# afermg/aliby

Measured on AMD Instinct MI355X. Metric: FOV tiles/sec (whole node), higher is better.
Workload: dtype u16 pixels, f64 feature accumulators, f32 dynamics, bfloat16 U-Net

## Files before the change

### aliby_amd/csrc/nn_conv.hip

```cpp
#include "common.h"
#include <utility>

typedef __bf16 bf16x8_t __attribute__((ext_vector_type(8)));
typedef float f32x16_t __attribute__((ext_vector_type(16)));
typedef float f32x2_t __attribute__((ext_vector_type(2)));

namespace {

template <class F, int... I>
__device__ __forceinline__ void static_for_impl(F&& f, std::integer_sequence<int, I...>) {
  (f(std::integral_constant<int, I>{}), ...);
}
template <int N, class F>
__device__ __forceinline__ void static_for(F&& f) {
  static_for_impl(static_cast<F&&>(f), std::make_integer_sequence<int, N>{});
}

__device__ __forceinline__ float cv_bf2f(unsigned h) { return __uint_as_float(h << 16); }
typedef __bf16 bf16x2_t __attribute__((ext_vector_type(2)));
__device__ __forceinline__ unsigned cv_pack2(float lo, float hi) {
  const f32x2_t f = {lo, hi};
  const bf16x2_t b = __builtin_convertvector(f, bf16x2_t);
  return __builtin_bit_cast(unsigned, b);
}
// ... 298 lines not shown
          const int gapi = kb < 32 ? kb + 1 : TW + 2;
          const int bp = lx - 1 - (lx > gapi ? 1 : 0);
          const int snd = bp >= kb ? 1 : 0;
          const int c = snd ? bp - kb : cst + bp;
          const bool ok = lx != gapi && c >= 0 && c < a.W && !(bp == TW && kb == TW) && (unsigned)gy < (unsigned)a.H;
          const int img = (snd && ok) ? g0 + 1 : g0;
          inside |= (unsigned)ok << u;
          later |= (unsigned)snd << u;
          v[u] = inN[(unsigned)(((img * a.H + cy) * IW + min(max(c, 0), a.W - 1)) * a.cs + pl)];
        } else {
          const int gxi = x0 - 1 + lx;
          inside |= (unsigned)((unsigned)gy < (unsigned)a.H && (unsigned)gxi < (unsigned)a.W) << u;
          const int cx = min(max(gxi, 0), a.W - 1);
          v[u] = inN[(unsigned)(((UP ? cy >> 1 : cy) * IW + (UP ? cx >> 1 : cx)) * a.cs + pl)];
        }
      }
#pragma unroll
      for (int u = 0; u < BATCH; ++u) {
        if (it0 + u >= ITERS) break;
        uint4 o;
        if constexpr (PACK) {
          f32x2_t shs[4];
#pragma unroll
          for (int k = 0; k < 4; ++k) shs[k] = ((later >> u) & 1u) ? sh1[k] : sh[k];
          o = conv_act8(v[u], sc, shs, 0u - ((inside >> u) & 1u));
        } else {
          o = conv_act8(v[u], sc, sh, 0u - ((inside >> u) & 1u));
        }
        if (it0 + u == ITERS - 1 && p0 + (it0 + u) * PIX_PER_IT >= RAW) continue;
        lds[pl * PLANE + p0 + (it0 + u) * PIX_PER_IT] = o;
      }
    }
    if constexpr (PK > 0) {
      constexpr int POCT = 2 * PK, PUNITS = TH * TW * POCT;
      const uint4* pN = a.pin + (size_t)n * a.H * a.W * a.pcs;
#pragma unroll
      for (int it = 0; it < (PUNITS + 255) / 256; ++it) {
        const int u = tid + it * 256;
        if (u >= PUNITS) break;
        const int oct = u % POCT, pix = u / POCT;
        const int cy = min(y0 + pix / TW, a.H - 1), cx = min(x0 + pix % TW, a.W - 1);
        uint4 v = make_uint4(0, 0, 0, 0);
        if (oct < a.pcs) v = pN[(unsigned)((cy * a.W + cx) * a.pcs + oct)];
        ldsP[oct * PPLANE + pix] = v;
      }
    }
    CONV_STAMP(3);
    __syncthreads();
    CONV_STAMP(4);

#pragma unroll
    for (int pass = 0; pass < PASSES; ++pass) {
      const int rbase = (rg * PASSES + pass) * R;
      f32x16_t acc[R];
      {
        float4 b4[4];
#pragma unroll
        for (int q = 0; q < 4; ++q) b4[q] = float4(sbias[(c0 >> 2) + q]);
        conv_seed<R>(acc, b4, rr, a.res != nullptr);
      }
      __builtin_amdgcn_sched_barrier(0);
      if (pass + 1 < PASSES && a.res) load_res(pass + 1);
      __builtin_amdgcn_sched_barrier(0);
      conv_mfma<R, KC, (POOL ? cfg::DEPTH_POOL : cfg::DEPTH), PLANE, LW>(
          reinterpret_cast<const bf16x8_t*>(lds) + hh * PLANE + rbase * LW + px + second, wfrag, acc);
      if constexpr (PK > 0) {
        const bf16x8_t* LP = reinterpret_cast<const bf16x8_t*>(ldsP) + hh * PPLANE + rbase * TW + px;
#pragma unroll
        for (int r = 0; r < R; ++r)
#pragma unroll
          for (int k = 0; k < PK; ++k)
            acc[r] = __builtin_amdgcn_mfma_f32_32x32x16_bf16(pfrag[k], LP[2 * k * PPLANE + r * TW], acc[r], 0, 0, 0);
      }
      if (pass == PASSES - 1) CONV_STAMP(5);
      if constexpr (HEAD) {
        __builtin_amdgcn_sched_barrier(0);
#pragma unroll
        for (int r = 0; r < R; ++r) {
          const f32x16_t y = head_from_acc(acc[r], hconst, hconst + 32, hwf, hh);
          const int gy = y0 + rbase + r;
          if (hh == 0 && gx < a.W && gy < a.H) {
            float* hp = a.hout + (size_t)n * a.hO * a.H * a.W + (size_t)gy * a.W + gx;
            const float yo[4] = {y[0], y[1], y[2], y[3]};
            for (int o = 0; o < a.hO; ++o) hp[(size_t)o * a.H * a.W] = yo[o] + hconst[64 + o];
          }
        }
      }
      if (!HEAD || a.out) conv_store<R>(a, nimg, irow, y0 + rbase, gx, c0, acc);
      if constexpr (POOL) {
        const int PH = a.H >> 1, PW = a.W >> 1;
#pragma unroll
        for (int r = 0; r < R; r += 2) {
          const int gy = y0 + rbase + r;
          const bool writer = (px & 1) == 0 && gx + 1 < a.W && gy + 1 < a.H;
          uint4* pp = a.pool + (size_t)nimg * PH * PW * a.ocs + a.ocoff + (unsigned)((((irow + gy) >> 1) * PW + (gx >> 1)) * a.ocs + (c0 >> 3));
#pragma unroll
          for (int half = 0; half < 2; ++half) {
            unsigned pk[4];
#pragma unroll
            for (int q = 0; q < 4; ++q) {
              const float v0 = fmaxf(acc[r][half * 8 + 2 * q], acc[r + 1][half * 8 + 2 * q]);
              const float v1 = fmaxf(acc[r][half * 8 + 2 * q + 1], acc[r + 1][half * 8 + 2 * q + 1]);
              pk[q] = cv_pack2(fmaxf(v0, __shfl_xor(v0, 1)), fmaxf(v1, __shfl_xor(v1, 1)));
            }
            if (writer) pp[half] = make_uint4(pk[0], pk[1], pk[2], pk[3]);
          }
        }
      }
    }
    CONV_STAMP(6);
  }
}

template <int CIN, int COUT, bool UP, bool PACK = false>
struct DmaCfg {
  static constexpr int KC = CIN / 16, NPL = CIN / 8, NCB = COUT / 32;
  static constexpr int WAVES_PER_SIMD = CIN >= 128 ? 1 : 2;
  static constexpr int R = CIN >= 64 ? 2 : 4;
  static constexpr int PASSES = (CIN >= 128 || COUT >= 128) ? 2 : 1;
  static constexpr int RG = 4 / NCB;
  static constexpr int TH = RG * R * PASSES, TW = 32, LH = TH + 2, LW = TW + 2 + (PACK ? 1 : 0);
  static constexpr int RAW = LH * LW;
  static constexpr int PLANE = NPL == 4 ? RAW + (10 - RAW % 8) % 8 : (RAW | 1);
  static constexpr int A_SLOTS = NPL * PLANE;
  static constexpr int PIX_PER_IT = 256 / NPL;
  static constexpr int ITERS = (RAW + PIX_PER_IT - 1) / PIX_PER_IT;
  static constexpr int RLH = UP ? TH / 2 + 2 : LH, RLW = UP ? TW / 2 + 2 : LW;
  static constexpr int RUNITS = RLH * RLW * NPL;
  static constexpr int GIT = (RUNITS + 255) / 256;
  static constexpr int R_SLOTS = GIT * 256;
  static constexpr int LDS_BYTES = (A_SLOTS + R_SLOTS) * 16;
  static constexpr int DEPTH = (CIN >= 64 && COUT >= 64) ? 4 : 6;
};

template <int CIN, int COUT, bool UP, bool PACK = false>
__global__ __launch_bounds__(256, (DmaCfg<CIN, COUT, UP, PACK>::WAVES_PER_SIMD)) void k_conv3x3_dma(ConvArgs a) {
  static_assert(!PACK || UP, "the packed LDS-DMA variant is written for upsampled input");
  using cfg = DmaCfg<CIN, COUT, UP, PACK>;
  constexpr int KC = cfg::KC, NPL = cfg::NPL, NCB = cfg::NCB, R = cfg::R, TH = cfg::TH, TW = cfg::TW;
  constexpr int LW = cfg::LW, RAW = cfg::RAW, PLANE = cfg::PLANE, RLW = cfg::RLW, PASSES = cfg::PASSES;
  constexpr int PIX_PER_IT = cfg::PIX_PER_IT, ITERS = cfg::ITERS, GIT = cfg::GIT;
  extern __shared__ uint4 lds[];
  uint4* const ldsA = lds;
  uint4* const ldsR = lds + cfg::A_SLOTS;

  const int tid = threadIdx.x, lane = tid & 63, wave = tid >> 6;
  const int cb = wave % NCB, rg = wave / NCB;
  const int px = lane & 31, hh = lane >> 5;
  const int c0 = cb * 32 + hh * 16;

  bf16x8_t wfrag[9 * KC];
  {
    const bf16x8_t* wp = reinterpret_cast<const bf16x8_t*>(a.wpk) + (size_t)cb * 9 * KC * 64 + lane;
#pragma unroll
    for (int i = 0; i < 9 * KC; ++i) wfrag[i] = wp[i * 64];
  }
  const int pl = tid % NPL, pix0 = tid / NPL;
  const int ly0 = pix0 / LW, lx0 = pix0 - ly0 * LW;
  f32x2_t sc[4];
#pragma unroll
  for (int k = 0; k < 4; ++k) sc[k] = f32x2_t{a.scale[pl * 8 + 2 * k], a.scale[pl * 8 + 2 * k + 1]};

  const int IH = UP ? a.H >> 1 : a.H, IW = UP ? a.W >> 1 : a.W;
  const int xcd = blockIdx.x & 7, slot = blockIdx.x >> 3, nslots = gridDim.x >> 3;
  const int per_xcd = (a.ntiles + 7) >> 3;
  const int t_end = min(a.ntiles, (xcd + 1) * per_xcd);
  const int wave_u = __builtin_amdgcn_readfirstlane(wave);

  auto issue_dma = [&](int tile) {
    const int tx = tile % a.tiles_x, tyn = tile / a.tiles_x;
    const int ty = tyn % a.tiles_y, n = tyn / a.tiles_y;
    const int ry0 = UP ? (ty * TH >> 1) - 1 : ty * TH - 1, rx0 = UP ? (tx * TW >> 1) - 1 : tx * TW - 1;
    int g0 = 0, cst = 0, half = 1 << 20;
    if constexpr (PACK) {
      g0 = (tx * TW) / a.W;
      cst = tx * TW - g0 * a.W;
      half = (a.W - cst) >> 1;
    }
    const uint4* inN = a.in + (size_t)(PACK ? n * a.G : n) * IH * IW * a.cs + a.coff;
    int t0 = tid;
    asm volatile("" : "+v"(t0));
#pragma unroll
    for (int k = 0; k < GIT; ++k) {
      const int unit = t0 + k * 256;
      const int rpix = unit / NPL, oct = unit % NPL;
      const int rly = rpix / RLW, rlx = rpix - rly * RLW;
      const int iy = min(max(ry0 + rly, 0), IH - 1);
      int ix, img = 0;
      if constexpr (PACK) {
        const bool first = rlx <= half;
        ix = min(max(first ? (cst >> 1) - 1 + rlx : rlx - half - 1, 0), IW - 1);
        img = first ? g0 : min(g0 + 1, a.G - 1);
      } else {
        ix = min(max(rx0 + rlx, 0), IW - 1);
      }
      const uint4* g = inN + (unsigned)(((img * IH + iy) * IW + ix) * a.cs + oct);
      __builtin_amdgcn_global_load_lds((const __attribute__((address_space(1))) void*)g,
                                       (__attribute__((address_space(3))) void*)(ldsR + k * 256 + wave_u * 64), 16, 0, 0);
    }
  };

  int tile = xcd * per_xcd + slot, stamp_tile = 0;
  if (tile < t_end) issue_dma(tile);
  for (; tile < t_end; tile += nslots, ++stamp_tile) {
    CONV_STAMP(0);
    const int tx = tile % a.tiles_x, tyn = tile / a.tiles_x;
    const int ty = tyn % a.tiles_y, n = tyn / a.tiles_y;
    const int y0 = ty * TH, x0 = tx * TW;
    int g0 = 0, cst = x0, kb = 1 << 20, nimg = n;
    if constexpr (PACK) {
      g0 = x0 / a.W;
      cst = x0 - g0 * a.W;
      kb = a.W - cst;
      nimg = n * a.G;
    }
    const int second = (PACK && px >= kb) ? 1 : 0;
    const int gx = PACK ? (second ? px - kb : cst + px) : x0 + px;
    const int irow = PACK ? (g0 + second) * a.H : 0;

    f32x2_t sh[4], sh1[PACK ? 4 : 1];
    {
      const float* sp = a.shift + (size_t)(nimg + g0) * a.shift_stride + pl * 8;
#pragma unroll
      for (int k = 0; k < 4; ++k) sh[k] = f32x2_t{sp[2 * k], sp[2 * k + 1]};
      if constexpr (PACK) {
        const float* sq = a.shift + (size_t)(nimg + min(g0 + 1, a.G - 1)) * a.shift_stride + pl * 8;
#pragma unroll
        for (int k = 0; k < 4; ++k) sh1[k] = f32x2_t{sq[2 * k], sq[2 * k + 1]};
      }
    }
    float4 b4[4] = {};
    if (a.bias) {
      const float4* bp = reinterpret_cast<const float4*>(a.bias + c0);
#pragma unroll
      for (int q = 0; q < 4; ++q) b4[q] = bp[q];
    }
    uint4 rr[R][2];
    auto load_res = [&](int pass) { conv_load_res<R>(a, nimg, irow, y0 + (rg * PASSES + pass) * R, gx, c0, rr); };
    if (a.res) load_res(0);
    CONV_STAMP(1);
    asm volatile("s_waitcnt vmcnt(0)" ::: "memory");
    __syncthreads();
    CONV_STAMP(2);
    {
      const int ry0 = UP ? (y0 >> 1) - 1 : y0 - 1, rx0 = UP ? (x0 >> 1) - 1 : x0 - 1;
      int p0 = pix0, qy = ly0, qx = lx0;
      asm volatile("" : "+v"(p0), "+v"(qy), "+v"(qx));
#pragma unroll
      for (int it = 0; it < ITERS; ++it) {
        int lx = qx + (it * PIX_PER_IT) % LW, ly = qy + (it * PIX_PER_IT) / LW;
        if (lx >= LW) { lx -= LW; ly += 1; }
        const int gy = y0 - 1 + ly, gxi = x0 - 1 + lx;
        const int pix = p0 + it * PIX_PER_IT;
        unsigned keep;
        int rpix;
        uint4 o;
        if constexpr (PACK) {
          const int gapi = kb < 32 ? kb + 1 : TW + 2;
          const int bp = lx - 1 - (lx > gapi ? 1 : 0);
          const int snd = bp >= kb ? 1 : 0;
          const int c = snd ? bp - kb : cst + bp;
          keep = 0u - (unsigned)(lx != gapi && c >= 0 && c < a.W && !(bp == TW && kb == TW) && (unsigned)gy < (unsigned)a.H);
          const int rcol = snd ? (kb >> 1) + 1 + (c >> 1) : ((cst + bp) >> 1) - ((cst >> 1) - 1);
          rpix = min(max(((gy >> 1) - ry0) * RLW + rcol, 0), cfg::RLH * RLW - 1);
          f32x2_t shs[4];
#pragma unroll
          for (int k = 0; k < 4; ++k) shs[k] = snd ? sh1[k] : sh[k];
          o = conv_act8(ldsR[rpix * NPL + pl], sc, shs, keep);
        } else {
          keep = 0u - (unsigned)((unsigned)gy < (unsigned)a.H && (unsigned)gxi < (unsigned)a.W);
          rpix = UP ? min(((gy >> 1) - ry0) * RLW + ((gxi >> 1) - rx0), cfg::RLH * RLW - 1) : min(pix, RAW - 1);
          o = conv_act8(ldsR[rpix * NPL + pl], sc, sh, keep);
        }
        if (it == ITERS - 1 && pix >= RAW) continue;
        ldsA[pl * PLANE + pix] = o;
      }
    }
    CONV_STAMP(3);
    __syncthreads();
#pragma unroll
    for (int pass = 0; pass < PASSES; ++pass) {
      const int rbase = (rg * PASSES + pass) * R;
      f32x16_t acc[R];
      conv_seed<R>(acc, b4, rr, a.res != nullptr);
      __builtin_amdgcn_sched_barrier(0);
      if (pass == 0 && tile + nslots < t_end) issue_dma(tile + nslots);
      if (pass + 1 < PASSES && a.res) load_res(pass + 1);
      __builtin_amdgcn_sched_barrier(0);
      if (pass == 0) CONV_STAMP(4);
      conv_mfma<R, KC, cfg::DEPTH, PLANE, LW>(reinterpret_cast<const bf16x8_t*>(ldsA) + hh * PLANE + rbase * LW + px + second, wfrag, acc);
      if (pass == PASSES - 1) CONV_STAMP(5);
      conv_store<R>(a, nimg, irow, y0 + rbase, gx, c0, acc);
    }
    CONV_STAMP(6);
  }
}

struct PairCfg {
  static constexpr int KC = 2, NPL = 4, R = 2, PASSES = 2;
  static constexpr int TH = 14, TWO = 30, MH = 16, MW = 32, IH = 18, IW = 34;
  static constexpr int RAW_IN = IH * IW, PLANE_IN = RAW_IN + (10 - RAW_IN % 8) % 8;
  static constexpr int RAW_MID = MH * MW, PLANE_MID = RAW_MID + (10 - RAW_MID % 8) % 8;
  static constexpr int PIX_PER_IT = 256 / NPL, ITERS = (RAW_IN + PIX_PER_IT - 1) / PIX_PER_IT;
  static constexpr int MID_SLOTS = NPL * PLANE_MID + 8;
  static constexpr int SLOTS = NPL * PLANE_IN + 2 * MID_SLOTS;
  static constexpr int LDS_BYTES = SLOTS * 16;
  static constexpr int DEPTH = 6;
};

template <bool POOL, bool HEAD>
__global__ __launch_bounds__(512, 1) void k_conv_pair32(ConvArgs a) {
  static_assert(!(POOL && HEAD), "either the pooled output (down block) or the output head (last unit)");
  using cfg = PairCfg;
  constexpr int KC = cfg::KC, NPL = cfg::NPL, R = cfg::R, PASSES = cfg::PASSES, TH = cfg::TH, TWO = cfg::TWO;
  constexpr int IW_ = cfg::IW, MW = cfg::MW, PLANE_IN = cfg::PLANE_IN, PLANE_MID = cfg::PLANE_MID, RAW_IN = cfg::RAW_IN;
  constexpr int PIX_PER_IT = cfg::PIX_PER_IT, ITERS = cfg::ITERS;
  extern __shared__ uint4 lds[];
  uint4* const ldsIn = lds;
  uint4* const ldsMid0 = lds + NPL * PLANE_IN;
  __shared__ __align__(16) float tabB[64];
  __shared__ float hconst[HEAD ? 2 * 32 + 4 : 1];

  const int consumer = threadIdx.x >> 8;
  const int tid = threadIdx.x & 255, lane = tid & 63, wave = tid >> 6;
  const int px = lane & 31, hh = lane >> 5;
  const int c0 = hh * 16;

  const int xcd = blockIdx.x & 7, slot = blockIdx.x >> 3, nslots = gridDim.x >> 3;
  const int per_xcd = (a.ntiles + 7) >> 3;
  const int t_begin = xcd * per_xcd + slot, t_end = min(a.ntiles, (xcd + 1) * per_xcd);
  const int my_tiles = t_begin < t_end ? (t_end - t_begin + nslots - 1) / nslots : 0;

  if (!consumer) {
    bf16x8_t wA[9 * KC];
    {
      const bf16x8_t* pa = reinterpret_cast<const bf16x8_t*>(a.wpk) + lane;
#pragma unroll
      for (int i = 0; i < 9 * KC; ++i) wA[i] = pa[i * 64];
    }
    const int pl = tid % NPL, pix0 = tid / NPL;
    const int ly0 = pix0 / IW_, lx0 = pix0 - ly0 * IW_;
    f32x2_t sc[4];
#pragma unroll
    for (int k = 0; k < 4; ++k) sc[k] = f32x2_t{a.scale[pl * 8 + 2 * k], a.scale[pl * 8 + 2 * k + 1]};
    uint4 v[ITERS];
    unsigned inside = 0;
    auto request = [&](int tile) {
      const int tx = tile % a.tiles_x, tyn = tile / a.tiles_x;
      const int ty = tyn % a.tiles_y, n = tyn / a.tiles_y;
      const int y0 = ty * TH, x0 = tx * TWO;
      const uint4* inN = a.in + (size_t)n * a.H * a.W * a.cs + a.coff;
      inside = 0;
#pragma unroll
      for (int u = 0; u < ITERS; ++u) {
        int lx = lx0 + (u * PIX_PER_IT) % IW_, ly = ly0 + (u * PIX_PER_IT) / IW_;
        if (lx >= IW_) { lx -= IW_; ly += 1; }
        const int gy = y0 - 2 + ly, gxi = x0 - 2 + lx;
        inside |= (unsigned)((unsigned)gy < (unsigned)a.H && (unsigned)gxi < (unsigned)a.W) << u;
        const int cy = min(max(gy, 0), a.H - 1), cx = min(max(gxi, 0), a.W - 1);
        v[u] = inN[(unsigned)((cy * a.W + cx) * a.cs + pl)];
      }
    };
    if (my_tiles > 0) request(t_begin);
    for (int it = 0; it < my_tiles; ++it) {
      const int tile = t_begin + it * nslots;
      const int tx = tile % a.tiles_x, tyn = tile / a.tiles_x;
      const int ty = tyn % a.tiles_y, n = tyn / a.tiles_y;
      const int y0 = ty * TH, x0 = tx * TWO;
      uint4* const ldsMid = ldsMid0 + (it & 1) * cfg::MID_SLOTS;
      f32x2_t sh[4];
      {
        const float* sp = a.shift + (size_t)n * a.shift_stride + pl * 8;
#pragma unroll
        for (int k = 0; k < 4; ++k) sh[k] = f32x2_t{sp[2 * k], sp[2 * k + 1]};
      }
      if (tid < 32) {
        tabB[tid] = a.scale2[tid];
        tabB[32 + tid] = a.shift2[(size_t)n * a.shift2_stride + tid];
      }
#pragma unroll
      for (int u = 0; u < ITERS; ++u) {
        const uint4 o = conv_act8(v[u], sc, sh, 0u - ((inside >> u) & 1u));
        if (u == ITERS - 1 && pix0 + u * PIX_PER_IT >= RAW_IN) continue;
        ldsIn[pl * PLANE_IN + pix0 + u * PIX_PER_IT] = o;
      }
      __syncthreads();
      if (it + 1 < my_tiles) request(tile + nslots);
      __builtin_amdgcn_sched_barrier(0);
#pragma unroll
      for (int pass = 0; pass < PASSES; ++pass) {
        const int mbase = (wave * PASSES + pass) * R;
        f32x16_t acc[R];
        {
          float4 b4[4] = {};
          if (a.bias) {
            const float4* bp = reinterpret_cast<const float4*>(a.bias + c0);
#pragma unroll
            for (int q = 0; q < 4; ++q) b4[q] = bp[q];
          }
#pragma unroll
          for (int r = 0; r < R; ++r)
#pragma unroll
            for (int q = 0; q < 4; ++q) { acc[r][4 * q] = b4[q].x; acc[r][4 * q + 1] = b4[q].y; acc[r][4 * q + 2] = b4[q].z; acc[r][4 * q + 3] = b4[q].w; }
        }
        __builtin_amdgcn_sched_barrier(0);
        conv_mfma<R, KC, cfg::DEPTH, PLANE_IN, IW_>(reinterpret_cast<const bf16x8_t*>(ldsIn) + hh * PLANE_IN + mbase * IW_ + px, wA, acc);
        __builtin_amdgcn_sched_barrier(0);
        const int mgx = x0 - 1 + px;
#pragma unroll
        for (int r = 0; r < R; ++r) {
          const int mgy = y0 - 1 + mbase + r;
          const unsigned keep = 0u - (unsigned)((unsigned)mgy < (unsigned)a.H && (unsigned)mgx < (unsigned)a.W);
#pragma unroll
          for (int half = 0; half < 2; ++half) {
            f32x2_t s2[4], h2[4];
            const float4* tp = reinterpret_cast<const float4*>(tabB + c0 + 8 * half);
            const float4 sa = tp[0], sb = tp[1], ha = tp[8], hb = tp[9];
            s2[0] = f32x2_t{sa.x, sa.y}; s2[1] = f32x2_t{sa.z, sa.w}; s2[2] = f32x2_t{sb.x, sb.y}; s2[3] = f32x2_t{sb.z, sb.w};
            h2[0] = f32x2_t{ha.x, ha.y}; h2[1] = f32x2_t{ha.z, ha.w}; h2[2] = f32x2_t{hb.x, hb.y}; h2[3] = f32x2_t{hb.z, hb.w};
            const uint4 raw = make_uint4(cv_pack2(acc[r][8 * half + 0], acc[r][8 * half + 1]), cv_pack2(acc[r][8 * half + 2], acc[r][8 * half + 3]),
                                         cv_pack2(acc[r][8 * half + 4], acc[r][8 * half + 5]), cv_pack2(acc[r][8 * half + 6], acc[r][8 * half + 7]));
            ldsMid[(2 * hh + half) * PLANE_MID + (mbase + r) * MW + px] = conv_act8(raw, s2, h2, keep);
          }
        }
      }
      __syncthreads();
    }
    __syncthreads();
    __syncthreads();
  } else {
    bf16x8_t wB[9 * KC];
    {
      const bf16x8_t* pb = reinterpret_cast<const bf16x8_t*>(a.wpk2) + lane;
#pragma unroll
      for (int i = 0; i < 9 * KC; ++i) wB[i] = pb[i * 64];
    }
    HeadW hwf;
    if constexpr (HEAD) {
      hwf = head_weights(a.hw, a.hO, lane);
      if (tid < 32) {
        hconst[tid] = a.hscale[tid];
        hconst[32 + tid] = a.hshift[tid];
        if (tid < 4) hconst[64 + tid] = tid < a.hO ? a.hbias[tid] : 0.f;
      }
    }
    float4 b4[4] = {};
    if (a.bias2) {
      const float4* bp = reinterpret_cast<const float4*>(a.bias2 + c0);
#pragma unroll
      for (int q = 0; q < 4; ++q) b4[q] = bp[q];
    }
    __syncthreads();
    __syncthreads();
    for (int it = 0; it < my_tiles; ++it) {
      const int tile = t_begin + it * nslots;
      const int tx = tile % a.tiles_x, tyn = tile / a.tiles_x;
      const int ty = tyn % a.tiles_y, n = tyn / a.tiles_y;
      const int y0 = ty * TH, x0 = tx * TWO;
      const uint4* const ldsMid = ldsMid0 + (it & 1) * cfg::MID_SLOTS;
      const int gx = (px < TWO && x0 + px < a.W) ? x0 + px : a.W;
#pragma unroll
      for (int pass = 0; pass < PASSES; ++pass) {
        const int rbase = (wave * PASSES + pass) * R;
        if (rbase < TH) {
          uint4 rr[R][2];
          if (a.res) conv_load_res<R>(a, n, 0, y0 + rbase, min(gx, a.W - 1), c0, rr);
          f32x16_t acc[R];
          conv_seed<R>(acc, b4, rr, a.res != nullptr);
          __builtin_amdgcn_sched_barrier(0);
          conv_mfma<R, KC, cfg::DEPTH, PLANE_MID, MW>(reinterpret_cast<const bf16x8_t*>(ldsMid) + hh * PLANE_MID + rbase * MW + px, wB, acc);
          if constexpr (HEAD) {
#pragma unroll
            for (int r = 0; r < R; ++r) {
              const f32x16_t y = head_from_acc(acc[r], hconst, hconst + 32, hwf, hh);
              const int gy = y0 + rbase + r;
              if (hh == 0 && gx < a.W && gy < a.H) {
                float* hp = a.hout + (size_t)n * a.hO * a.H * a.W + (size_t)gy * a.W + gx;
                const float yo[4] = {y[0], y[1], y[2], y[3]};
                for (int o = 0; o < a.hO; ++o) hp[(size_t)o * a.H * a.W] = yo[o] + hconst[64 + o];
              }
            }
          }
          if (!HEAD || a.out) conv_store<R>(a, n, 0, y0 + rbase, gx, c0, acc);
          if constexpr (POOL) {
            const int PH = a.H >> 1, PW = a.W >> 1;
            const int gy = y0 + rbase;
            const bool writer = (px & 1) == 0 && gx + 1 < a.W && gy + 1 < a.H;
            uint4* pp = a.pool + (size_t)n * PH * PW * a.ocs + a.ocoff + (unsigned)(((gy >> 1) * PW + (min(gx, a.W - 1) >> 1)) * a.ocs + (c0 >> 3));
#pragma unroll
            for (int half = 0; half < 2; ++half) {
              unsigned pk[4];
#pragma unroll
              for (int q = 0; q < 4; ++q) {
                const float v0 = fmaxf(acc[0][half * 8 + 2 * q], acc[1][half * 8 + 2 * q]);
                const float v1 = fmaxf(acc[0][half * 8 + 2 * q + 1], acc[1][half * 8 + 2 * q + 1]);
                pk[q] = cv_pack2(fmaxf(v0, __shfl_xor(v0, 1)), fmaxf(v1, __shfl_xor(v1, 1)));
              }
              if (writer) pp[half] = make_uint4(pk[0], pk[1], pk[2], pk[3]);
            }
          }
        }
        __syncthreads();
      }
    }
  }
}

struct FirstPairCfg {
  static constexpr int KC = 2, NPL = 4, R = 2, PASSES = 2;
  static constexpr int TH = 14, TWO = 30, MH = 16, MW = 32, AH = 18, AW = 36;
  static constexpr int RAW_MID = MH * MW, PLANE_MID = RAW_MID + (10 - RAW_MID % 8) % 8;
  static constexpr int MID_SLOTS = NPL * PLANE_MID + 8;
  static constexpr int P0_WORDS = 2 * AH * AW;
  static constexpr int RAWP_WORDS = MH * MW;
  static constexpr int VALS = 2 * AH * AW, ITERS = (VALS + 255) / 256;
  static constexpr int LDS_BYTES = 2 * MID_SLOTS * 16 + P0_WORDS * 4 + 2 * RAWP_WORDS * 4;
  static constexpr int DEPTH = 6;
};

__global__ __launch_bounds__(512, 1) void k_conv_first_pair(ConvArgs a) {
  using cfg = FirstPairCfg;
  constexpr int KC = cfg::KC, R = cfg::R, PASSES = cfg::PASSES, TH = cfg::TH, TWO = cfg::TWO, MW = cfg::MW;
  constexpr int AH = cfg::AH, AW = cfg::AW, PLANE_MID = cfg::PLANE_MID, ITERS = cfg::ITERS;
  extern __shared__ uint4 lds[];
  uint4* const ldsMid0 = lds;
  unsigned* const P0 = reinterpret_cast<unsigned*>(lds + 2 * cfg::MID_SLOTS);
  unsigned* const rawP0 = P0 + cfg::P0_WORDS;
  __shared__ __align__(16) float tabB[64];

  const int consumer = threadIdx.x >> 8;
  const int tid = threadIdx.x & 255, lane = tid & 63, wave = tid >> 6;
  const int px = lane & 31, hh = lane >> 5;
  const int c0 = hh * 16;

  const int xcd = blockIdx.x & 7, slot = blockIdx.x >> 3, nslots = gridDim.x >> 3;
  const int per_xcd = (a.ntiles + 7) >> 3;
  const int t_begin = xcd * per_xcd + slot, t_end = min(a.ntiles, (xcd + 1) * per_xcd);
  const int my_tiles = t_begin < t_end ? (t_end - t_begin + nslots - 1) / nslots : 0;
  const size_t plane = (size_t)a.H * a.W;

  if (!consumer) {
    bf16x8_t wF[2];
    {
      const int m = lane & 31, co = 16 * ((m >> 2) & 1) + (m & 3) + 4 * (m >> 3);
#pragma unroll
      for (int kc = 0; kc < 2; ++kc) {
        unsigned r4[4];
#pragma unroll
        for (int j2 = 0; j2 < 4; ++j2) {
          float v[2];
#pragma unroll
          for (int e = 0; e < 2; ++e) {
            const int k = 16 * kc + 8 * hh + 2 * j2 + e, c = k / 12, ty = (k % 12) / 4, tx = k % 4;
            v[e] = (c < a.fcin && tx < 3 && k < 24) ? a.fw[((size_t)co * a.fcin + c) * 9 + ty * 3 + tx] : 0.f;
          }
          r4[j2] = cv_pack2(v[0], v[1]);
        }
        wF[kc] = __builtin_bit_cast(bf16x8_t, make_uint4(r4[0], r4[1], r4[2], r4[3]));
      }
    }
    int goff[2][2];
    unsigned gmask[2][2];
#pragma unroll
    for (int kc = 0; kc < 2; ++kc)
#pragma unroll
      for (int g = 0; g < 2; ++g) {
        const int k = 16 * kc + 8 * hh + 4 * g;
        const bool live = k < 24 && k / 12 < a.fcin;
        goff[kc][g] = live ? (k / 12) * AH * AW + ((k % 12) / 4) * AW : 0;
        gmask[kc][g] = live ? 0xffffffffu : 0u;
      }
    if (tid < 32) {
      tabB[tid] = a.scale2[tid];
      tabB[32 + tid] = a.shift2[tid];
    }
    const float fs0 = a.fscale[0], fh0 = a.fshift[0];
    const float fs1 = a.fcin > 1 ? a.fscale[1] : 0.f, fh1 = a.fcin > 1 ? a.fshift[1] : 0.f;
    float v[ITERS];
    unsigned inside = 0;
    auto request = [&](int tile) {
      const int tx = tile % a.tiles_x, tyn = tile / a.tiles_x;
      const int ty = tyn % a.tiles_y, n = tyn / a.tiles_y;
      const int y0 = ty * TH, x0 = tx * TWO;
      inside = 0;
#pragma unroll
      for (int u = 0; u < ITERS; ++u) {
        const int i = tid + 256 * u;
        const int c = i / (AH * AW), rem = i - c * (AH * AW), r = rem / AW, q = rem - r * AW;
        const int gy = y0 - 2 + r, gx = x0 - 2 + q;
        const bool ok = i < cfg::VALS && c < a.fcin && (unsigned)gy < (unsigned)a.H && (unsigned)gx < (unsigned)a.W;
        inside |= (unsigned)ok << u;
        const int cy = min(max(gy, 0), a.H - 1), cx = min(max(gx, 0), a.W - 1), cc = min(c, a.fcin - 1);
        v[u] = a.fx[((size_t)n * a.fcin + cc) * plane + (size_t)cy * a.W + cx];
      }
    };
    if (my_tiles > 0) request(t_begin);
    unsigned short* const P0h = reinterpret_cast<unsigned short*>(P0);
    for (int it = 0; it < my_tiles; ++it) {
      const int tile = t_begin + it * nslots;
      const int tx = tile % a.tiles_x, tyn = tile / a.tiles_x;
      const int ty = tyn % a.tiles_y;
      const int y0 = ty * TH, x0 = tx * TWO;
      uint4* const ldsMid = ldsMid0 + (it & 1) * cfg::MID_SLOTS;
      unsigned short* const rawPh = reinterpret_cast<unsigned short*>(rawP0 + (it & 1) * cfg::RAWP_WORDS);
#pragma unroll
      for (int u = 0; u < ITERS; ++u) {
        const int i = tid + 256 * u;
        if (i >= cfg::VALS) break;
        const int c = i / (AH * AW), rem = i - c * (AH * AW), r = rem / AW, q = rem - r * AW;
        const bool ok = (inside >> u) & 1u;
        const float t = ok ? fmaxf(v[u] * (c ? fs1 : fs0) + (c ? fh1 : fh0), 0.f) : 0.f;
        const unsigned short b = (unsigned short)(cv_pack2(t, 0.f) & 0xffffu);
        P0h[2 * i] = b;
        if (q > 0) P0h[2 * (i - 1) + 1] = b;
        if (q == AW - 1) P0h[2 * i + 1] = 0;
        if (r >= 2 && q >= 2 && q < 2 + MW)
          rawPh[2 * ((r - 2) * MW + (q - 2)) + c] = (unsigned short)(cv_pack2(ok ? v[u] : 0.f, 0.f) & 0xffffu);
      }
      if (a.fcin < 2) {
        for (int i = tid; i < cfg::RAWP_WORDS; i += 256) rawPh[2 * i + 1] = 0;
      }
      __syncthreads();
      if (it + 1 < my_tiles) request(tile + nslots);
      __builtin_amdgcn_sched_barrier(0);
#pragma unroll
      for (int pass = 0; pass < PASSES; ++pass) {
        const int mbase = (wave * PASSES + pass) * R;
        const int mgx = x0 - 1 + px;
#pragma unroll
        for (int r = 0; r < R; ++r) {
          const int m = mbase + r;
          f32x16_t acc;
#pragma unroll
          for (int k = 0; k < 16; ++k) acc[k] = 0.f;
#pragma unroll
          for (int kc = 0; kc < 2; ++kc) {
            const unsigned* w0 = P0 + goff[kc][0] + m * AW + px;
            const unsigned* w1 = P0 + goff[kc][1] + m * AW + px;
            const uint4 bfrag = make_uint4(w0[0] & gmask[kc][0], w0[2] & gmask[kc][0], w1[0] & gmask[kc][1], w1[2] & gmask[kc][1]);
            acc = __builtin_amdgcn_mfma_f32_32x32x16_bf16(wF[kc], __builtin_bit_cast(bf16x8_t, bfrag), acc, 0, 0, 0);
          }
          const int mgy = y0 - 1 + m;
          const unsigned keep = 0u - (unsigned)((unsigned)mgy < (unsigned)a.H && (unsigned)mgx < (unsigned)a.W);
#pragma unroll
          for (int half = 0; half < 2; ++half) {
            f32x2_t s2[4], h2[4];
            const float4* tp = reinterpret_cast<const float4*>(tabB + c0 + 8 * half);
            const float4 sa = tp[0], sb = tp[1], ha = tp[8], hb = tp[9];
            s2[0] = f32x2_t{sa.x, sa.y}; s2[1] = f32x2_t{sa.z, sa.w}; s2[2] = f32x2_t{sb.x, sb.y}; s2[3] = f32x2_t{sb.z, sb.w};
            h2[0] = f32x2_t{ha.x, ha.y}; h2[1] = f32x2_t{ha.z, ha.w}; h2[2] = f32x2_t{hb.x, hb.y}; h2[3] = f32x2_t{hb.z, hb.w};
            const uint4 raw = make_uint4(cv_pack2(acc[8 * half + 0], acc[8 * half + 1]), cv_pack2(acc[8 * half + 2], acc[8 * half + 3]),
                                         cv_pack2(acc[8 * half + 4], acc[8 * half + 5]), cv_pack2(acc[8 * half + 6], acc[8 * half + 7]));
            ldsMid[(2 * hh + half) * PLANE_MID + m * MW + px] = conv_act8(raw, s2, h2, keep);
          }
        }
      }
      __syncthreads();
    }
    __syncthreads();
    __syncthreads();
  } else {
    bf16x8_t wB[9 * KC];
    {
      const bf16x8_t* pb = reinterpret_cast<const bf16x8_t*>(a.wpk2) + lane;
#pragma unroll
      for (int i = 0; i < 9 * KC; ++i) wB[i] = pb[i * 64];
    }
    const bf16x8_t pfrag = (reinterpret_cast<const bf16x8_t*>(a.pwpk) + lane)[0];
    float4 b4[4] = {};
    if (a.bias2) {
      const float4* bp = reinterpret_cast<const float4*>(a.bias2 + c0);
#pragma unroll
      for (int q = 0; q < 4; ++q) b4[q] = bp[q];
    }
    __syncthreads();
    __syncthreads();
    for (int it = 0; it < my_tiles; ++it) {
      const int tile = t_begin + it * nslots;
      const int tx = tile % a.tiles_x, tyn = tile / a.tiles_x;
      const int ty = tyn % a.tiles_y, n = tyn / a.tiles_y;
      const int y0 = ty * TH, x0 = tx * TWO;
      const uint4* const ldsMid = ldsMid0 + (it & 1) * cfg::MID_SLOTS;
      const unsigned* const rawP = rawP0 + (it & 1) * cfg::RAWP_WORDS;
      const int gx = (px < TWO && x0 + px < a.W) ? x0 + px : a.W;
#pragma unroll
      for (int pass = 0; pass < PASSES; ++pass) {
        const int rbase = (wave * PASSES + pass) * R;
        if (rbase < TH) {
          f32x16_t acc[R];
#pragma unroll
          for (int r = 0; r < R; ++r)
#pragma unroll
            for (int q = 0; q < 4; ++q) { acc[r][4 * q] = b4[q].x; acc[r][4 * q + 1] = b4[q].y; acc[r][4 * q + 2] = b4[q].z; acc[r][4 * q + 3] = b4[q].w; }
          __builtin_amdgcn_sched_barrier(0);
          conv_mfma<R, KC, cfg::DEPTH, PLANE_MID, MW>(reinterpret_cast<const bf16x8_t*>(ldsMid) + hh * PLANE_MID + rbase * MW + px, wB, acc);
#pragma unroll
          for (int r = 0; r < R; ++r) {
            const unsigned w = hh ? 0u : rawP[(rbase + r) * MW + px];
            acc[r] = __builtin_amdgcn_mfma_f32_32x32x16_bf16(pfrag, __builtin_bit_cast(bf16x8_t, make_uint4(w, 0u, 0u, 0u)), acc[r], 0, 0, 0);
          }
          conv_store<R>(a, n, 0, y0 + rbase, gx, c0, acc);
        }
        __syncthreads();
      }
    }
  }
}

__global__ __launch_bounds__(256) void k_out_head_mfma(const uint4* __restrict__ x, const float* __restrict__ scale, const float* __restrict__ shift,
                                                       const float* __restrict__ w, const float* __restrict__ bias, int O, size_t N, size_t P,
                                                       float* __restrict__ out) {
  __shared__ float hconst[2 * 32 + 4];
  const int tid = threadIdx.x, lane = tid & 63, px = lane & 31, hh = lane >> 5;
  if (tid < 32) {
    hconst[tid] = scale[tid];
    hconst[32 + tid] = shift[tid];
    if (tid < 4) hconst[64 + tid] = tid < O ? bias[tid] : 0.f;
  }
  const HeadW hwf = head_weights(w, O, lane);
  __syncthreads();
  const size_t total = N * P, nblk = (total + 31) / 32;
  const size_t wave0 = ((size_t)blockIdx.x * blockDim.x + tid) >> 6, nwaves = ((size_t)gridDim.x * blockDim.x) >> 6;
  for (size_t b = wave0; b < nblk; b += nwaves) {
    const size_t pix = b * 32 + px;
    const bool ok = pix < total;
    const size_t q = ok ? pix : total - 1;
    const uint4 lo = x[q * 4 + 2 * hh], hi = x[q * 4 + 2 * hh + 1];
    const f32x16_t y = head_apply(lo, hi, hconst, hconst + 32, hwf, hh);
    if (ok && hh == 0) {
      const size_t n = pix / P, p = pix - n * P;
      const float yo[4] = {y[0], y[1], y[2], y[3]};
      for (int o = 0; o < O; ++o) out[(n * O + o) * P + p] = yo[o] + hconst[64 + o];
    }
  }
}

__global__ void k_pack_conv3x3(const float* w, int cout, int cin_src, int cin, int taps, unsigned short* out, size_t total) {
  const size_t i = (size_t)blockIdx.x * blockDim.x + threadIdx.x;
  if (i >= total) return;
  const int j = (int)(i & 7), lane = (int)((i >> 3) & 63);
  size_t rest = i >> 9;
  const int kcn = cin / 16;
  const int kc = (int)(rest % kcn);
  rest /= kcn;
  const int tap = (int)(rest % taps), cb = (int)(rest / taps);
  const int m = lane & 31, h = lane >> 5;
  const int co = cb * 32 + 16 * ((m >> 2) & 1) + (m & 3) + 4 * (m >> 3);
  const int ci = 16 * kc + 8 * h + j;
  float v = 0.f;
  if (ci < cin_src && co < cout) v = w[((size_t)co * cin_src + ci) * taps + tap];
  out[i] = (unsigned short)cv_f2bf(v);
}

unsigned long long* g_conv_trace = nullptr;

template <int CIN, int COUT, bool UP, bool PACK = false>
int launch_conv_dma(aliby_ctx* ctx, ConvArgs& a, hipStream_t stream) {
  using cfg = DmaCfg<CIN, COUT, UP, PACK>;
  a.G = PACK ? 224 / a.W : 1;
  a.tiles_x = PACK ? 224 / cfg::TW : (a.W + cfg::TW - 1) / cfg::TW;
  a.tiles_y = (a.H + cfg::TH - 1) / cfg::TH;
  const long long nt = (long long)(a.N / a.G) * a.tiles_x * a.tiles_y;
  ARG_CHECK(nt < INT_MAX, "conv3x3: too many tiles");
  a.ntiles = (int)nt;
  static bool attr_done = false;
  if (!attr_done) {
    HIP_TRY(hipFuncSetAttribute(reinterpret_cast<const void*>(&k_conv3x3_dma<CIN, COUT, UP, PACK>),
                                hipFuncAttributeMaxDynamicSharedMemorySize, cfg::LDS_BYTES));
    attr_done = true;
  }
  const int per_xcd = (a.ntiles + 7) / 8;
  const int cap = 32 * cfg::WAVES_PER_SIMD;
  const int nslots = per_xcd < cap ? per_xcd : cap;
  hipLaunchKernelGGL((k_conv3x3_dma<CIN, COUT, UP, PACK>), dim3(8 * nslots), dim3(256), cfg::LDS_BYTES, stream, a);
  KERNEL_CHECK();
  return ALIBY_OK;
}

template <int CIN, int COUT, bool UP, bool TALL, bool PACK = false>
int launch_conv_reg(aliby_ctx* ctx, ConvArgs& a, hipStream_t stream) {
  using cfg = ConvCfg<CIN, COUT, TALL, PACK>;
  a.G = PACK ? 224 / a.W : 1;
  a.tiles_x = PACK ? 224 / cfg::TW : (a.W + cfg::TW - 1) / cfg::TW;
  a.tiles_y = (a.H + cfg::TH - 1) / cfg::TH;
  const long long nt = (long long)(a.N / a.G) * a.tiles_x * a.tiles_y;
  ARG_CHECK(nt < INT_MAX, "conv3x3: too many tiles");
  a.ntiles = (int)nt;
  static bool attr_done = false;
  constexpr int PKV = PACK ? 0 : (!UP && CIN == 32 && COUT == 32) ? 1 : ((!UP && CIN == 64 && COUT == 64) ? 2 : 0);
  constexpr int P_BYTES = PKV ? 2 * PKV * ((cfg::TH * cfg::TW) | 1) * 16 : 0;
  if (!attr_done) {
    HIP_TRY(hipFuncSetAttribute(reinterpret_cast<const void*>(&k_conv3x3<CIN, COUT, UP, false, 0, TALL, PACK>),
                                hipFuncAttributeMaxDynamicSharedMemorySize, cfg::LDS_BYTES));
    HIP_TRY(hipFuncSetAttribute(reinterpret_cast<const void*>(&k_conv3x3<CIN, COUT, UP, true, 0, TALL, PACK>),
                                hipFuncAttributeMaxDynamicSharedMemorySize, cfg::LDS_BYTES));
    if constexpr (PKV > 0)
      HIP_TRY(hipFuncSetAttribute(reinterpret_cast<const void*>(&k_conv3x3<CIN, COUT, UP, false, PKV, TALL>),
                                  hipFuncAttributeMaxDynamicSharedMemorySize, cfg::LDS_BYTES + P_BYTES));
    attr_done = true;
  }
  const int per_xcd = (a.ntiles + 7) / 8;
  const int nslots = per_xcd < 64 ? per_xcd : 64;
  if (a.pin) {
    if constexpr (PKV > 0) {
      ARG_CHECK(!a.pool && a.pcs >= 1 && a.pcs <= 2 * PKV, "conv3x3: fused projection: unsupported input width");
// ... 264 lines not shown
```

Before: 614.7.

## Double-buffer input window and prefetch residuals across tiles in conv pair kernel

The producer half now double-buffers the activated input window in LDS. It stages tile it+1 while computing tile it and requests tile it+2, so each tile needs one barrier instead of two. Per-tile scale/shift values are loaded once per lane and spread with shuffles, and the bias moves into LDS. The consumer half prefetches residual rows for the next pass or tile into rotating registers and drops the per-pass barrier. The cost is twice the LDS for the input window, extra register pressure, and a shallower MFMA pipeline depth (DEPTH_A) on the first conv.

Measured after the change: 619.4 (median of 6 runs). Within noise of the previous version (+0.8%).

```diff
diff --git a/aliby_amd/csrc/nn_conv.hip b/aliby_amd/csrc/nn_conv.hip
--- a/aliby_amd/csrc/nn_conv.hip
+++ b/aliby_amd/csrc/nn_conv.hip
@@ -624,10 +624,12 @@
   static constexpr int RAW_IN = IH * IW, PLANE_IN = RAW_IN + (10 - RAW_IN % 8) % 8;
   static constexpr int RAW_MID = MH * MW, PLANE_MID = RAW_MID + (10 - RAW_MID % 8) % 8;
   static constexpr int PIX_PER_IT = 256 / NPL, ITERS = (RAW_IN + PIX_PER_IT - 1) / PIX_PER_IT;
+  static constexpr int WIN_SLOTS = NPL * PLANE_IN;
   static constexpr int MID_SLOTS = NPL * PLANE_MID + 8;
-  static constexpr int SLOTS = NPL * PLANE_IN + 2 * MID_SLOTS;
+  static constexpr int SLOTS = 2 * WIN_SLOTS + 2 * MID_SLOTS;
   static constexpr int LDS_BYTES = SLOTS * 16;
   static constexpr int DEPTH = 6;
+  static constexpr int DEPTH_A = 5;
 };
 
 template <bool POOL, bool HEAD>
@@ -638,9 +640,10 @@
   constexpr int IW_ = cfg::IW, MW = cfg::MW, PLANE_IN = cfg::PLANE_IN, PLANE_MID = cfg::PLANE_MID, RAW_IN = cfg::RAW_IN;
   constexpr int PIX_PER_IT = cfg::PIX_PER_IT, ITERS = cfg::ITERS;
   extern __shared__ uint4 lds[];
-  uint4* const ldsIn = lds;
-  uint4* const ldsMid0 = lds + NPL * PLANE_IN;
-  __shared__ __align__(16) float tabB[64];
+  uint4* const ldsIn0 = lds;
+  uint4* const ldsMid0 = lds + 2 * cfg::WIN_SLOTS;
+  __shared__ __align__(16) float tabB[2][64];
+  __shared__ __align__(16) float biasA[32];
   __shared__ float hconst[HEAD ? 2 * 32 + 4 : 1];
 
   const int consumer = threadIdx.x >> 8;
@@ -661,17 +664,22 @@
       for (int i = 0; i < 9 * KC; ++i) wA[i] = pa[i * 64];
     }
     const int pl = tid % NPL, pix0 = tid / NPL;
-    const int ly0 = pix0 / IW_, lx0 = pix0 - ly0 * IW_;
-    f32x2_t sc[4];
-#pragma unroll
-    for (int k = 0; k < 4; ++k) sc[k] = f32x2_t{a.scale[pl * 8 + 2 * k], a.scale[pl * 8 + 2 * k + 1]};
+    const float scl = a.scale[tid & 31];
+    if (tid < 32) {
+      biasA[tid] = a.bias ? a.bias[tid] : 0.f;
+      tabB[0][tid] = tabB[1][tid] = a.scale2[tid];
+    }
     uint4 v[ITERS];
+    float shl, tb;
     unsigned inside = 0;
     auto request = [&](int tile) {
       const int tx = tile % a.tiles_x, tyn = tile / a.tiles_x;
       const int ty = tyn % a.tiles_y, n = tyn / a.tiles_y;
       const int y0 = ty * TH, x0 = tx * TWO;
       const uint4* inN = a.in + (size_t)n * a.H * a.W * a.cs + a.coff;
+      int p0 = pix0;
+      asm volatile("" : "+v"(p0));
+      const int ly0 = p0 / IW_, lx0 = p0 - ly0 * IW_;
       inside = 0;
 #pragma unroll
       for (int u = 0; u < ITERS; ++u) {
@@ -682,51 +690,59 @@
         const int cy = min(max(gy, 0), a.H - 1), cx = min(max(gxi, 0), a.W - 1);
         v[u] = inN[(unsigned)((cy * a.W + cx) * a.cs + pl)];
       }
+      shl = a.shift[(size_t)n * a.shift_stride + (tid & 31)];
+      tb = a.shift2[(size_t)n * a.shift2_stride + (tid & 31)];
     };
-    if (my_tiles > 0) request(t_begin);
-    for (int it = 0; it < my_tiles; ++it) {
-      const int tile = t_begin + it * nslots;
-      const int tx = tile % a.tiles_x, tyn = tile / a.tiles_x;
-      const int ty = tyn % a.tiles_y, n = tyn / a.tiles_y;
-      const int y0 = ty * TH, x0 = tx * TWO;
-      uint4* const ldsMid = ldsMid0 + (it & 1) * cfg::MID_SLOTS;
-      f32x2_t sh[4];
-      {
-        const float* sp = a.shift + (size_t)n * a.shift_stride + pl * 8;
-#pragma unroll
-        for (int k = 0; k < 4; ++k) sh[k] = f32x2_t{sp[2 * k], sp[2 * k + 1]};
-      }
-      if (tid < 32) {
-        tabB[tid] = a.scale2[tid];
-        tabB[32 + tid] = a.shift2[(size_t)n * a.shift2_stride + tid];
-      }
+    auto stage = [&](int b) {
+      if (tid < 32) tabB[b][32 + tid] = tb;
+      f32x2_t sc[4], sh[4];
+#pragma unroll
+      for (int k = 0; k < 4; ++k) {
+        sc[k] = f32x2_t{__shfl(scl, pl * 8 + 2 * k), __shfl(scl, pl * 8 + 2 * k + 1)};
+        sh[k] = f32x2_t{__shfl(shl, pl * 8 + 2 * k), __shfl(shl, pl * 8 + 2 * k + 1)};
+      }
+      uint4* const ldsIn = ldsIn0 + b * cfg::WIN_SLOTS;
 #pragma unroll
       for (int u = 0; u < ITERS; ++u) {
         const uint4 o = conv_act8(v[u], sc, sh, 0u - ((inside >> u) & 1u));
         if (u == ITERS - 1 && pix0 + u * PIX_PER_IT >= RAW_IN) continue;
         ldsIn[pl * PLANE_IN + pix0 + u * PIX_PER_IT] = o;
       }
-      __syncthreads();
-      if (it + 1 < my_tiles) request(tile + nslots);
+    };
+    const int t_last = t_begin + (my_tiles - 1) * nslots;
+    if (my_tiles > 0) {
+      request(t_begin);
+      stage(0);
+      request(min(t_begin + nslots, t_last));
+    }
+    __syncthreads();
+    for (int it = 0; it < my_tiles; ++it) {
+      const int tile = t_begin + it * nslots;
+      const int tx = tile % a.tiles_x, tyn = tile / a.tiles_x;
+      const int ty = tyn % a.tiles_y;
+      const int y0 = ty * TH, x0 = tx * TWO;
+      const uint4* const ldsIn = ldsIn0 + (it & 1) * cfg::WIN_SLOTS;
+      uint4* const ldsMid = ldsMid0 + (it & 1) * cfg::MID_SLOTS;
+      const float* const tab = tabB[it & 1];
+      if (it + 1 < my_tiles) stage((it + 1) & 1);
+      request(min(tile + 2 * nslots, t_last));
       __builtin_amdgcn_sched_barrier(0);
 #pragma unroll
       for (int pass = 0; pass < PASSES; ++pass) {
         const int mbase = (wave * PASSES + pass) * R;
         f32x16_t acc[R];
         {
-          float4 b4[4] = {};
-          if (a.bias) {
-            const float4* bp = reinterpret_cast<const float4*>(a.bias + c0);
-#pragma unroll
-            for (int q = 0; q < 4; ++q) b4[q] = bp[q];
-          }
+          float4 b4[4];
+          const float4* bp = reinterpret_cast<const float4*>(biasA + c0);
+#pragma unroll
+          for (int q = 0; q < 4; ++q) b4[q] = bp[q];
 #pragma unroll
           for (int r = 0; r < R; ++r)
 #pragma unroll
             for (int q = 0; q < 4; ++q) { acc[r][4 * q] = b4[q].x; acc[r][4 * q + 1] = b4[q].y; acc[r][4 * q + 2] = b4[q].z; acc[r][4 * q + 3] = b4[q].w; }
         }
         __builtin_amdgcn_sched_barrier(0);
-        conv_mfma<R, KC, cfg::DEPTH, PLANE_IN, IW_>(reinterpret_cast<const bf16x8_t*>(ldsIn) + hh * PLANE_IN + mbase * IW_ + px, wA, acc);
+        conv_mfma<R, KC, cfg::DEPTH_A, PLANE_IN, IW_>(reinterpret_cast<const bf16x8_t*>(ldsIn) + hh * PLANE_IN + mbase * IW_ + px, wA, acc);
         __builtin_amdgcn_sched_barrier(0);
         const int mgx = x0 - 1 + px;
 #pragma unroll
@@ -736,7 +752,7 @@
 #pragma unroll
           for (int half = 0; half < 2; ++half) {
             f32x2_t s2[4], h2[4];
-            const float4* tp = reinterpret_cast<const float4*>(tabB + c0 + 8 * half);
+            const float4* tp = reinterpret_cast<const float4*>(tab + c0 + 8 * half);
             const float4 sa = tp[0], sb = tp[1], ha = tp[8], hb = tp[9];
             s2[0] = f32x2_t{sa.x, sa.y}; s2[1] = f32x2_t{sa.z, sa.w}; s2[2] = f32x2_t{sb.x, sb.y}; s2[3] = f32x2_t{sb.z, sb.w};
             h2[0] = f32x2_t{ha.x, ha.y}; h2[1] = f32x2_t{ha.z, ha.w}; h2[2] = f32x2_t{hb.x, hb.y}; h2[3] = f32x2_t{hb.z, hb.w};
@@ -748,8 +764,6 @@
       }
       __syncthreads();
     }
-    __syncthreads();
-    __syncthreads();
   } else {
     bf16x8_t wB[9 * KC];
     {
@@ -772,7 +786,34 @@
 #pragma unroll
       for (int q = 0; q < 4; ++q) b4[q] = bp[q];
     }
-    __syncthreads();
+    const uint4* const resp = a.res ? a.res + a.ocoff : a.in + a.coff;
+    auto load_res = [&](int tile, int pass, uint4 (&rr)[R][2]) {
+      const int tx = tile % a.tiles_x, tyn = tile / a.tiles_x;
+      const int ty = tyn % a.tiles_y, n = tyn / a.tiles_y;
+      const int cx = min(tx * TWO + min(px, TWO - 1), a.W - 1);
+      const uint4* resN = resp + (size_t)n * a.H * a.W * a.ocs;
+#pragma unroll
+      for (int r = 0; r < R; ++r) {
+        const int cy = min(ty * TH + (wave * PASSES + pass) * R + r, a.H - 1);
+        const unsigned off = (unsigned)((cy * a.W + cx) * a.ocs + (c0 >> 3));
+        rr[r][0] = resN[off];
+        rr[r][1] = resN[off + 1];
+      }
+    };
+    auto settle = [](uint4 (&rr)[R][2]) {
+#pragma unroll
+      for (int r = 0; r < R; ++r)
+#pragma unroll
+        for (int k = 0; k < 2; ++k) asm volatile("" : "+v"(rr[r][k].x), "+v"(rr[r][k].y), "+v"(rr[r][k].z), "+v"(rr[r][k].w));
+    };
+#pragma unroll
+    for (int q = 0; q < 4; ++q) asm volatile("" : "+v"(b4[q].x), "+v"(b4[q].y), "+v"(b4[q].z), "+v"(b4[q].w));
+#pragma unroll
+    for (int i = 0; i < 9 * KC; ++i) asm volatile("" : "+v"(wB[i]));
+    const int t_last = t_begin + (my_tiles - 1) * nslots;
+    uint4 rr0[R][2], rr1[R][2];
+    if (my_tiles > 0) load_res(t_begin, 0, rr0);
+    settle(rr0);
     __syncthreads();
     for (int it = 0; it < my_tiles; ++it) {
       const int tile = t_begin + it * nslots;
@@ -781,16 +822,21 @@
       const int y0 = ty * TH, x0 = tx * TWO;
       const uint4* const ldsMid = ldsMid0 + (it & 1) * cfg::MID_SLOTS;
       const int gx = (px < TWO && x0 + px < a.W) ? x0 + px : a.W;
+      __syncthreads();
 #pragma unroll
       for (int pass = 0; pass < PASSES; ++pass) {
         const int rbase = (wave * PASSES + pass) * R;
+        uint4 (&rr)[R][2] = pass == 0 ? rr0 : rr1;
+        __builtin_amdgcn_sched_barrier(0);
+        if (pass == 0) load_res(tile, 1, rr1);
+        else load_res(min(tile + nslots, t_last), 0, rr0);
+        __builtin_amdgcn_sched_barrier(0);
         if (rbase < TH) {
-          uint4 rr[R][2];
-          if (a.res) conv_load_res<R>(a, n, 0, y0 + rbase, min(gx, a.W - 1), c0, rr);
           f32x16_t acc[R];
           conv_seed<R>(acc, b4, rr, a.res != nullptr);
           __builtin_amdgcn_sched_barrier(0);
           conv_mfma<R, KC, cfg::DEPTH, PLANE_MID, MW>(reinterpret_cast<const bf16x8_t*>(ldsMid) + hh * PLANE_MID + rbase * MW + px, wB, acc);
+          settle(pass == 0 ? rr1 : rr0);
           if constexpr (HEAD) {
 #pragma unroll
             for (int r = 0; r < R; ++r) {
@@ -821,8 +867,9 @@
               if (writer) pp[half] = make_uint4(pk[0], pk[1], pk[2], pk[3]);
             }
           }
+        } else {
+          settle(rr0);
         }
-        __syncthreads();
       }
     }
   }
```
